# okgarces/deep-successor-features-for-transfer

Measured on AMD Instinct MI355X. Metric: env steps/sec (whole node), Reacher 8-task SF-DQN at 1/2/4/8 MI355X, higher is better.
Workload: dtype fp32; 1 GPU; reacher17-all-T8-B32 (Reacher-shape |s|=17 |a|=7 d=8, psi MLP 256x2, all heads updated per env step: main_sfdqn_torch.py path); heads_per_gpu=8, heads_total=8, global_batch=32, replay=host, parallelism=single

## Files before the change

deep-successor-features-for-transfer_amd/csrc/sfx.hip:

```cpp
#include <hip/hip_ext.h>
#include <hip/hip_runtime.h>
#include <dlfcn.h>
#include <rccl/rccl.h>

#include <cmath>
#include <cstdio>
#include <cstdlib>
#include <cstring>
#include <algorithm>
#include <atomic>
#include <chrono>
#include <deque>
#include <map>
#include <random>
#include <string>
#include <functional>
#include <tuple>
#include <utility>
#include <vector>

#include "sfx_kernels.h"
#include "sfx_gpiw.h"
#include "sfx_tsf.h"
#include "sfx_phi.h"
// ... 140 lines not shown
    const float *S = nullptr, *S1 = nullptr, *phi = nullptr, *gamma = nullptr, *s_next = nullptr;
    const int64_t* a = nullptr;
    float* losses = nullptr;
    bool pre = false;
    const float* ax = nullptr;
    int aM = 0;
    bool posted = false;
    float* q_out = nullptr;
    int64_t* task_out = nullptr;
    const unsigned long long* out_ind = nullptr;
  } pend;
  long long steps_spec = 0, steps_fallback = 0, policies_rerun = 0, rounds_total = 0;
  long long graph_captures = 0, graph_launches = 0;
  int force_rerun_from = -1;
  int spec_rounds = 2;
  bool spec_rounds_auto = true;
  int Tg = 0, off = 0;
  struct sfx_tsf_state* tsf = nullptr;
  struct sfx_phi_state* phi = nullptr;
  int comm_rank = 0, comm_world = 0;
  ncclComm_t comm = nullptr;
  bool comm_owned = false;
  ncclComm_t comm_rounds = nullptr;
  bool rounds_comm = false;
  bool comm_dead = false;
  std::string comm_err;
  long long* dstall = nullptr;
  bool comm_force = false;
  int (*host_ar)(void*, int32_t*, int) = nullptr;
  void* host_ar_ctx = nullptr;
  int32_t* host_ar_buf = nullptr;
  size_t host_ar_cap = 0;
  int *xb[2] = {nullptr, nullptr}, *xge = nullptr;
  int *tsx = nullptr, *tsz = nullptr;
  int *qh = nullptr, *qhs = nullptr;
  bool shard_qa = true;
  struct ShardPending {
    bool active = false;
    int B = 0;
    const float *S = nullptr, *S1 = nullptr, *phi = nullptr, *gamma = nullptr, *s_next = nullptr;
    const int64_t* a = nullptr;
  } spend;

  float *online = nullptr, *target = nullptr, *am = nullptr, *av = nullptr;
  float *w = nullptr, *wm = nullptr, *wv = nullptr;
  int* step = nullptr;
  int* dcancel = nullptr;
  AdamC* adamc = nullptr;
  float *act = nullptr, *dz = nullptr, *rowloss = nullptr;
  int64_t* spec_next = nullptr;
  int* skip = nullptr;
  unsigned long long* skipc = nullptr;
  bool skip_rounds = true;
  StepOut* dout = nullptr;
  HostResult* pub_res = nullptr;
  const long long* pub_dctr = nullptr;
  bool pub_folded = false;
  bool fold_publish = true;
  bool bf16 = false;
  __bf16* on16 = nullptr;
  __bf16* tg16 = nullptr;
  int dxs_max = 1, dx_ntile = 1;
  float* dxpart = nullptr;
  unsigned* dxctr = nullptr;
  StepOut* hout = nullptr;
  bool post_hout = false, hout_posted = false;
  unsigned long long* xin = nullptr;
  hipEvent_t ev_step = nullptr;
  unsigned long long gen = 0;
  int in_runner = 0;

  int slot(int head) const { return (int)((mask >> head) & 1ull); }
  unsigned long long all_bits() const { return T >= 64 ? ~0ull : ((1ull << T) - 1ull); }
  float* online_cur(int head) const { return online + ((size_t)slot(head) * T + head) * P; }
  float* am_cur(int head) const { return am + ((size_t)slot(head) * T + head) * P; }
  float* av_cur(int head) const { return av + ((size_t)slot(head) * T + head) * P; }
  float* target_of(int head) const { return target + (size_t)head * P; }
  __bf16* on16_cur(int head) const { return on16 + ((size_t)slot(head) * T + head) * P; }
  __bf16* tg16_of(int head) const { return tg16 + (size_t)head * P; }
};

namespace {

inline void touch(sfx_handle* h) {
  if (!h->in_runner) ++h->gen;
}

void clear_graphs(sfx_handle* h) {
  for (auto& kv : h->graphs) (void)hipGraphExecDestroy(kv.second);
  h->graphs.clear();
  h->graph_posts.clear();
}

enum { K_FWD = 0, K_TDG = 1, K_BWD = 2, K_GPI = 3, K_LMS = 4, K_VER = 5, K_TSF = 6, K_NKIND = 7 };

hipEvent_t prof_event(sfx_handle* h) {
  if (!h->prof_pool.empty()) {
    hipEvent_t e = h->prof_pool.back();
    h->prof_pool.pop_back();
    return e;
  }
  hipEvent_t e = nullptr;
  (void)hipEventCreate(&e);
  return e;
}

// ... 342 lines not shown
  A.tdg_next = td.next;
  A.tdg_xmax = td.xmax;
  A.tdg_poloff = td.poloff;
  A.flag = td.flag;
  A.flag_value = h->T;
  A.dz_scale = td.dz_scale;
  if (armed && fuse) {
    A.tdg_prev = td.prev;
    A.skip = h->skip;
    A.skipc = h->skipc;
    A.skip_v0 = ex.skip_fwd ? 1 : 0;
  }
  if (armed) {
    A.skip = h->skip;
    A.skip_v0 = ex.skip_fwd ? 1 : 0;
  }
  if (ex.skip_armed) *ex.skip_armed = armed;
  const int tail_at = fuse ? 1 : 0;
  const bool need_tail = losses || r || !fuse;
  const double tdg_bytes = 4.0 * nhead * M * ((td.use_gpi ? h->T : 1) * h->O + 2.0 * h->O + 2.0 * h->d + 4);
  A.M = M;
  A.head0 = head0;
  A.mask = h->mask;
  A.hp = h->hp_psi;
  A.hpw = h->hp_w;
  A.x0 = x0;
  A.phi = phi;
  A.r = r;
  A.train_w = r != nullptr;
  A.losses = losses;
  A.inc_step = ex.inc_step;
  auto dw_tiles = [&](int l) { return cdiv(h->L[l].N, 32) * cdiv(h->L[l].K, 64); };
  auto geo = [&](int l) {
    const LayerGeo& L = h->L[l];
    RoleGeo r{};
    r.N = L.N;
    r.K = L.K;
    r.wOff = L.wOff;
    r.bOff = L.bOff;
    r.actIn = L.actIn;
    r.xOff = l == 0 ? -1 : h->actOff[l - 1];
    r.dzOff = h->actOff[l];
    r.dzIn = l == 0 ? 0 : h->actOff[l - 1];
    return r;
  };
  auto dx_bytes = [&](int l) {
    const LayerGeo& L = h->L[l];
    return 4.0 * ((double)L.N * L.K + (double)M * L.N + 2.0 * M * L.K);
  };
  auto dw_bytes = [&](int l) {
    const LayerGeo& L = h->L[l];
    return 24.0 * ((double)L.N * L.K + L.N) + 4.0 * ((double)M * L.N + (double)M * L.K);
  };
  for (int l = h->NL - 1; l >= 1; --l) {
    const int li = h->NL - 1 - l;
    A.tdg = fuse && li == 0 ? 1 : 0;
    A.xi_src = A.tdg ? td.xi_src : nullptr;
    A.xi_dst = A.tdg ? td.xi_dst : nullptr;
    A.xi_copy = td.xi_copy;
    A.xi_n = td.xi_n;
    const double by = nhead * (dx_bytes(l) + (l + 1 <= h->NL - 1 ? dw_bytes(l + 1) : 0.0)) + (A.tdg ? tdg_bytes : 0.0);
    A.ra = geo(l);
    A.na = cdiv(M, 32) * cdiv(h->L[l].K, 16);
    A.dxs = 1;
    if (!A.tdg && h->dxpart && h->L[l].N > DX_SPLIT_N && M <= 32 * cdiv(h->Mmax, 32) &&
        nhead <= h->T) {
      A.dxs = cdiv(h->L[l].N, DX_SPLIT_N);
      A.dxpart = h->dxpart;
      A.dxctr = h->dxctr;
      A.na *= A.dxs;
    }
    if (l + 1 <= h->NL - 1) {
      A.rb = geo(l + 1);
      A.nb = dw_tiles(l + 1);
    } else {
      A.nb = 0;
    }
    A.nc = 0;
    A.tail = li == tail_at && need_tail ? 1 : 0;
    const int ntile = A.tdg ? A.na : A.na + A.nb + A.nc + A.tail;
    const dim3 grid = A.xcd ? dim3(8 * cdiv(nhead, 8) * ntile) : dim3(ntile, nhead);
    if (A.tdg && tdg_variant(h) == 1)
      launch(h, K_BWD, by, k_bwd_tdg<2, 8>, grid, dim3(256), h->G, A);
    else if (A.tdg)
      launch(h, K_BWD, by, k_bwd_tdg<4, 4>, grid, dim3(256), h->G, A);
    else if (!(ex.ride && nhead == 1 && !A.xcd && ex.ride(li, tail_at, A, ntile, by)))
      launch(h, K_BWD, by, h->bf16 ? k_bwd<true> : k_bwd<false>, grid, dim3(256), h->G, A);
  }
  A.na = 0;
  A.dxs = 1;
  A.tdg = 0;
  A.xi_dst = nullptr;
  A.xi_src = nullptr;
  A.rb = geo(1);
  A.nb = dw_tiles(1);
  A.rc = geo(0);
  A.nc = dw_tiles(0);
  A.tail = h->NL - 1 == tail_at && need_tail ? 1 : 0;
  A.fuse_v0 = ex.fuse_v0 ? 1 : 0;
  A.vM = M + (ex.v_xn ? 1 : 0);
  A.vOff = h->actOff[0];
  A.vRole = ex.vRole;
  A.act0 = h->L[0].actOut;
  A.v_x = ex.v_x;
  A.v_xn = ex.v_xn;
  A.ax = ex.fuse_v0 ? ex.ax : nullptr;
  A.aM = ex.fuse_v0 && ex.ax ? ex.aM : 0;
  A.a_noskip = ex.a_noskip;
  const int ntile = A.nb + A.nc + A.tail;
  if (!(ex.ride && nhead == 1 && !A.xcd && ex.ride(h->NL - 1, tail_at, A, ntile, nhead * (dw_bytes(1) + dw_bytes(0)))))
    launch(h, K_BWD, nhead * (dw_bytes(1) + dw_bytes(0)), h->bf16 ? k_bwd<true> : k_bwd<false>,
           A.xcd ? dim3(8 * cdiv(nhead, 8) * ntile) : dim3(ntile, nhead), dim3(256), h->G, A);
  LAUNCHCHK();
  return SFX_OK;
}

GpiArgs gpi_args(int role, int rowoff, int row0, const float* w, float* psi, float* q, int64_t* task, int64_t* next,
                 int64_t* sel, int select_task, int use_gpi, int M) {
  GpiArgs A{};
  A.M = M;
  A.role = role;
  A.row0 = row0;
  A.rowoff = rowoff;
  A.select_task = select_task;
  A.use_gpi = use_gpi;
  A.w = w;
  A.psi_out = psi;
  A.q_out = q;
  A.task_out = task;
  A.next_out = next;
  A.sel_out = sel;
  return A;
}

int run_gpi(sfx_handle* h, const GpiArgs& A) {
  launch(h, K_GPI, 4.0 * A.M * ((double)h->T * h->O * (A.psi_out ? 2 : 1) + h->d + (A.q_out ? h->T * h->A : 0)),
         k_gpi, dim3(A.M), dim3(256), h->G, A);
  LAUNCHCHK();
  return SFX_OK;
}

int run_ver(sfx_handle* h, int M, int npol, bool sel, int post, const GpiArgs& g, const int64_t* spec,
            bool post_host = false) {
  VerArgs V{};
  V.M = M;
  V.post = post;
  V.npol = npol;
  V.sel = sel ? 1 : 0;
  V.spec_stride = MMAX;
  V.spec_next = spec;
  V.flag = &h->dout->flag;
  V.g = g;
  const int TA = h->T * h->A;
  V.rows = TA >= 256 ? 1 : (256 / TA < M ? 256 / TA : M);
  const bool wide = wide_gpi(h) && npol > 1;
  const dim3 grid = wide ? dim3(M, cdiv(npol, WPC) + 1) : dim3(npol + 1, cdiv(M, V.rows));
  if (sel && h->pub_res && h->fold_publish) {
    V.pub = h->pub_res;
    V.pub_dctr = h->pub_dctr;
    V.done = &h->dout->done;
    V.nblocks = (int)(grid.x * grid.y);
    h->pub_folded = true;
  } else if (post_host) {
    V.h_sel = h->hout->sel;
// ... 483 lines not shown
  unsigned n = 0;
  if (hipDeviceSynchronize() != hipSuccess) return -1;
  if (hipMemcpyFromSymbol(&n, HIP_SYMBOL(sfx::g_probe_n), sizeof(n)) != hipSuccess) return -1;
  if (n > sfx::PROBE_N) n = sfx::PROBE_N;
  if ((int)n > max_recs) n = (unsigned)max_recs;
  if (n && hipMemcpyFromSymbol(out_host, HIP_SYMBOL(sfx::g_probe), n * sizeof(sfx::ProbeRec)) != hipSuccess) return -1;
  const unsigned z = 0;
  if (hipMemcpyToSymbol(HIP_SYMBOL(sfx::g_probe_n), &z, sizeof(z)) != hipSuccess) return -1;
  return (int)n;
}
#endif

int sfx_create(sfx_t* out, int T, int n_s, int H, int n_hidden, const int* acts, int A, int d, int max_batch,
               int device, void* stream) {
  if (!out) SFX_FAIL(SFX_E_ARG, "out is null");
  *out = nullptr;
  if (T < 1 || T > 64 || n_s < 1 || H < 1 || n_hidden < 0 || n_hidden + 2 > NLMAX || A < 1 || d < 1 ||
      max_batch < 1)
    SFX_FAIL(SFX_E_ARG, "bad geometry (1 <= T <= 64 heads per handle)");
  if (d > DMAX || max_batch + 1 > MMAX || (long)T * A > QMAX || (long)A * d > OMAX)
    SFX_FAIL(SFX_E_ARG, "geometry exceeds kernel limits (d<=256, batch<1024, T*A<=8192, A*d<=4096)");
  for (int i = 0; i < n_hidden; ++i)
    if (!acts || acts[i] < ACT_NONE || acts[i] > ACT_TANH) SFX_FAIL(SFX_E_ARG, "bad activation code");
  HIPCHK(hipSetDevice(device));
  sfx_handle* h = new sfx_handle();
  h->T = T;
  h->n_s = n_s;
  h->H = H;
  h->nh = n_hidden;
  h->A = A;
  h->d = d;
  h->O = A * d;
  h->NL = n_hidden + 2;
  h->Mmax = max_batch;
  h->device = device;
  h->stream = (hipStream_t)stream;
  h->dpad = align4(d);
  const char* eg = std::getenv("SFX_GRAPHS");
  h->use_graphs = !(eg && eg[0] == '0');
  const char* efp = std::getenv("SFX_FOLD_PUBLISH");
  h->fold_publish = !(efp && efp[0] == '0');
  {
    int dev = 0, ncu = 0;
    if (hipGetDevice(&dev) == hipSuccess &&
        hipDeviceGetAttribute(&ncu, hipDeviceAttributeMultiprocessorCount, dev) == hipSuccess && ncu > 0)
      h->ncu = ncu;
  }
  const char* etp = std::getenv("SFX_FWD_TPW");
  h->fwd_tpw = etp && etp[0] == '1' ? 1 : FWD_TPW;
  const char* eqa = std::getenv("SFX_SHARD_QA");
  h->shard_qa = !(eqa && eqa[0] == '0');
  const char* esk = std::getenv("SFX_SKIP");
  h->skip_rounds = !(esk && esk[0] == '0');
  int off = 0, ptorch = 0;
  for (int l = 0; l < h->NL; ++l) {
    LayerGeo Lr{};
    if (l == 0) {
      Lr.N = H; Lr.K = n_s; Lr.actOut = ACT_NONE;
    } else if (l == h->NL - 1) {
      Lr.N = h->O; Lr.K = H; Lr.actOut = ACT_NONE;
    } else {
      Lr.N = H; Lr.K = H; Lr.actOut = acts[l - 1];
    }
    Lr.actIn = l > 0 ? h->L[l - 1].actOut : ACT_NONE;
    Lr.wOff = align8(off);
    off = Lr.wOff + Lr.N * Lr.K;
    Lr.bOff = align4(off);
    off = Lr.bOff + Lr.N;
    ptorch += Lr.N * Lr.K + Lr.N;
    h->L.push_back(Lr);
  }
  h->P = (off + 63) & ~63;
  h->Ptorch = ptorch;
  int aoff = 0;
  for (int l = 0; l < h->NL; ++l) {
    h->actOff.push_back(aoff);
    aoff += align4((max_batch + 1) * h->L[l].N);
  }
  h->actSize = (aoff + 63) & ~63;
  h->Tg = T;
  h->spec_rounds = auto_spec_rounds(T);
  h->since_target.assign(T, 0);
  h->host_step.assign(T, 0);

  const size_t headBytes = sizeof(float) * (size_t)T * h->P;
  const size_t wBytes = sizeof(float) * (size_t)T * h->dpad;
  int rc = SFX_OK;
  auto alloc = [&](void** p, size_t bytes) {
    if (rc != SFX_OK) return;
    if (hipMalloc(p, bytes) != hipSuccess || hipMemset(*p, 0, bytes) != hipSuccess) {
      g_err = "hipMalloc failed";
      rc = SFX_E_HIP;
    }
  };
  alloc((void**)&h->online, 2 * headBytes);
  alloc((void**)&h->target, headBytes);
  alloc((void**)&h->am, 2 * headBytes);
  alloc((void**)&h->av, 2 * headBytes);
  alloc((void**)&h->w, wBytes);
  alloc((void**)&h->wm, wBytes);
  alloc((void**)&h->wv, wBytes);
  alloc((void**)&h->step, sizeof(int) * T);
  alloc((void**)&h->dcancel, 64);
  alloc((void**)&h->adamc, sizeof(AdamC) * T);
  {
    int nmax = 0, kmax = 0;
// ... 655 lines not shown
```

deep-successor-features-for-transfer_amd/csrc/sfx_kernels.h:

```cpp
#pragma once
#include <hip/hip_runtime.h>
#include <stdint.h>

#include <type_traits>

namespace sfx {

typedef float floatx4 __attribute__((ext_vector_type(4)));

constexpr int NLMAX = 8;
constexpr int MT = 32;
constexpr int QMAX = 8192;
constexpr int OMAX = 4096;
constexpr int DMAX = 256;
constexpr int MMAX = 1024;
constexpr int KFUSE = 64;
constexpr int GEMV_N = 512;
constexpr int GEMV_M = 4;
constexpr int DX_SPLIT_N = 256;
constexpr int VFUSE = 4096;
constexpr int TQF = 4096;

enum { ACT_NONE = 0, ACT_RELU = 1, ACT_TANH = 2 };
enum { R_S = 0, R_S1T = 1, R_S1 = 2, R_G = 3, R_A = 4, R_V = 5, R_V2 = 6, R_NS = 7, R_NS1T = 8, R_NS1 = 9, NROLE = 10 };
// ... 957 lines not shown
  float* grow = G.dzp(pol, NLm) + (size_t)b * O;
  const float* crow = G.actp(R_S, pol, NLm) + (size_t)b * O;
  const int an = s_next;
  for (int o = tid; o < O; o += 256) {
    float gv = 0.f;
    if (aok && o >= ab * d && o < ab * d + d) {
      const int k = o - ab * d;
      const float tg = __fadd_rn(A.phi[(size_t)b * d + k], __fmul_rn(gam, s_t[an * d + k]));
      gv = td_grad(G.huber, norm, __fsub_rn(crow[o], tg));
    }
    grow[o] = gv;
  }
  float dsq = 0.f;
  if (tid < d && aok) {
    const float diff = __fsub_rn(cval, __fadd_rn(phik, __fmul_rn(gam, s_t[an * d + tid])));
    dsq = td_loss(G.huber, diff);
    if (!__builtin_isfinite(diff) && G.nonfin) atomicOr(G.nonfin, 1);
  }
  if (tid < d) s_sq[tid] = dsq;
  __syncthreads();
  if (tid == 0) {
    float s = 0.f;
    for (int k = 0; k < d; ++k) s = __fadd_rn(s, s_sq[k]);
    SFX_CHK(pol >= 0 && pol < G.T && b < MMAX, pol, b, 0);
    G.rowloss[(long long)pol * MMAX + b] = s;
  }
  PROBE_REC(17, pt0);
}

struct RoleGeo {
  int N, K, wOff, bOff, actIn;
  int xOff;
  int dzOff;
  int dzIn;
};

struct BwdArgs {
  int M, na, nb, nc, tail, head0, train_w, inc_step;
  int xcd, nhead;
  int step_in_tail;
  int tdg, tdg_use_gpi, tdg_guess, tdg_next_stride, flag_value, pad2_;
  const int64_t* tdg_a;
  const float* tdg_gamma;
  int64_t* tdg_next;
  const int* tdg_xmax;
  int tdg_poloff, pad3_;
  int* flag;
  int fuse_v0, vM, vOff, act0;
  int vRole, dxs;
  unsigned long long mask;
  float* dxpart;
  unsigned* dxctr;
  RoleGeo ra, rb, rc;
  AdamHP hp, hpw;
  const float* x0;
  const float* phi;
  const float* r;
  float* losses;
  const float* v_x;
  const float* v_xn;
  const float* ax;
  int aM, a_noskip;
  const int* xi_src;
  int* xi_dst;
  int xi_copy, xi_n;
  const int64_t* tdg_prev;
  int* skip;
  unsigned long long* skipc;
  int skip_v0, pad4_;
  const float* dz_scale;
};

__device__ __forceinline__ const float* layer_input(const Geo& G, const BwdArgs& A, int head, int xOff) {
  return xOff < 0 ? A.x0 : G.actp(R_S, head, xOff);
}

constexpr int TDG_ROWS_O = 128;
struct TdgSmem {
  float w[32], gam[32], ph[32 * 16];
  int a[32], n[32];
  float q[2048], m[32 * 128];
  float tt[32 * TDG_ROWS_O], tc[32 * TDG_ROWS_O];
  float dz[32 * TDG_ROWS_O];
};

template <int VMAX, int U, bool C>
__device__ int tdg_rows(const Geo& G, const BwdArgs& A, int pol, int m0, bool pub, TdgSmem& sm) {
  const int tid = threadIdx.x, T = G.T, Aa = G.A, d = G.d, O = G.O, NLm = G.lastOff, M = A.M;
  const int nb = M - m0 < 32 ? M - m0 : 32;
  const bool xm = A.tdg_xmax != nullptr;
  const int t0 = A.tdg_use_gpi ? 0 : pol, nt = A.tdg_use_gpi ? T : 1, TA = nt * Aa, n = xm ? 0 : nb * TA, V = d >> 2;
  const int guess = A.tdg_guess;
  const FDiv fTA = fdiv(TA), fA = fdiv(Aa);
  float4 v[U][VMAX];
#pragma unroll
  for (int u = 0; u < U; ++u) {
    const int idx = tid + u * 256;
    const bool ok = idx < n;
    const int bl = idx / fTA, rem = idx - bl * TA, tq = rem / fA, t = t0 + tq, a = rem - tq * Aa;
    const float4* p = reinterpret_cast<const float4*>(G.actp(t < pol ? guess : R_S1, ok ? t : 0, NLm) +
                                                      (ok ? (size_t)(m0 + bl) * O + a * d : 0));
#pragma unroll
    for (int j = 0; j < VMAX; ++j) v[u][j] = (ok && j < V) ? p[j] : make_float4(0.f, 0.f, 0.f, 0.f);
  }
  const int n4 = (nb * O) >> 2;
  const float4* tg4 = reinterpret_cast<const float4*>(G.actp(R_S1T, pol, NLm) + (size_t)m0 * O);
  const float4* cu4 = reinterpret_cast<const float4*>(G.actp(R_S, pol, NLm) + (size_t)m0 * O);
  float4 tt[4], tc[4];
#pragma unroll
  for (int u = 0; u < 4; ++u) {
    const int i = tid + u * 256;
    tt[u] = i < n4 ? tg4[i] : make_float4(0.f, 0.f, 0.f, 0.f);
    tc[u] = i < n4 ? cu4[i] : make_float4(0.f, 0.f, 0.f, 0.f);
  }
  const int np4 = (nb * d) >> 2;
  const float4 ph = tid < np4 ? reinterpret_cast<const float4*>(A.phi + (size_t)m0 * d)[tid] : make_float4(0.f, 0.f, 0.f, 0.f);
  const float wk = tid < d ? G.w[(long long)pol * G.dpad + tid] : 0.f;
  const int ab_l = tid < nb ? (int)A.tdg_a[m0 + tid] : 0;
  const float gam_l = tid < nb ? A.tdg_gamma[m0 + tid] : 0.f;
  int xv[4];
  if (xm) {
    const int* xr = A.tdg_xmax + ((size_t)(A.tdg_poloff + pol) * M + m0) * Aa;
// ... 67 lines not shown
    if (pub && A.tdg_next) A.tdg_next[(size_t)(pol - A.head0) * A.tdg_next_stride + m0 + bl] = am;
  }
  const int same = !__syncthreads_or(differs);
  if (pub && A.skip && tid == 0) {
    A.skip[pol] = same;
    if (A.skipc && prev) {
      atomicAdd(A.skipc, 1ull);
      if (same) atomicAdd(A.skipc + 1, 1ull);
    }
  }
  if (same) return 1;
  PROBE_AT(4);
  const float norm = td_norm(G, M, O, A.dz_scale);
  const FDiv fd = fdiv(d);
  float* sq = sm.q;
  int nf = 0;
  for (int i = tid; i < nb * d; i += 256) {
    const int bl = i / fd, k = i - bl * d, ab = sm.a[bl];
    float e2 = 0.f;
    if (ab >= 0 && ab < Aa) {
      const float tg = __fadd_rn(sm.ph[bl * d + k], __fmul_rn(sm.gam[bl], sm.tt[bl * O + sm.n[bl] * d + k]));
      const float diff = __fsub_rn(sm.tc[bl * O + ab * d + k], tg);
      sm.dz[bl * O + ab * d + k] = td_grad(G.huber, norm, diff);
      e2 = td_loss(G.huber, diff);
      nf |= !__builtin_isfinite(diff);
    }
    sq[i] = e2;
  }
  if (__syncthreads_or(nf) && tid == 0 && G.nonfin) atomicOr(G.nonfin, 1);
  PROBE_AT(7);
  if (pub) {
    float4* gout4 = reinterpret_cast<float4*>(G.dzp(pol, NLm) + (size_t)m0 * O);
    for (int i = tid; i < n4; i += 256) {
      const float4 v = reinterpret_cast<const float4*>(sm.dz)[i];
      if constexpr (C) {
        float* o = reinterpret_cast<float*>(gout4 + i);
        stc<true>(o, v.x);
        stc<true>(o + 1, v.y);
        stc<true>(o + 2, v.z);
        stc<true>(o + 3, v.w);
      } else {
        gout4[i] = v;
      }
    }
    for (int bl = tid; bl < nb; bl += 256) {
      float sacc = 0.f;
      for (int k = 0; k < d; ++k) sacc = __fadd_rn(sacc, sq[bl * d + k]);
      SFX_CHK(pol >= 0 && pol < G.T && m0 + bl < MMAX, pol, m0 + bl, 0);
      G.rowloss[(long long)pol * MMAX + m0 + bl] = sacc;
    }
  }
  PROBE_AT(8);
  return 0;
}

template <bool TDG, int VMAX = 2, int U = 8, bool C = false, bool BF = false>
__device__ __forceinline__ void role_dx(const Geo& G, const BwdArgs& A, int head, int tile, floatx4 (*red)[2][64]) {
  static_assert(!(BF && (TDG || C)), "bf16 dX: the plain dX tiles only (the fused TD launch stays fp32)");
  const RoleGeo L = A.ra;
  const int N = L.N, K = L.K, M = A.M;
  const int ntk = (K + 15) >> 4;
  const int split = TDG ? 0 : tile % A.dxs;
  tile = TDG ? tile : tile / A.dxs;
  const int nchunk = ((N + A.dxs - 1) / A.dxs + 63) & ~63;
  const int nbeg = split * nchunk, nend = min(N, nbeg + nchunk);
  const int k0 = (tile % ntk) * 16, m0 = (tile / ntk) * 32;
  const int wave = threadIdx.x >> 6, lane = threadIdx.x & 63, r = lane & 15, g = lane >> 4;
  const float* W = G.online + G.slot_off(rslot(A.mask, head), head) + L.wOff;
  const float* Xin = layer_input(G, A, head, L.xOff);
  float* out = G.dzp(head, L.dzIn);
  const int ma = m0 + r, mb = m0 + 16 + r, kk = k0 + r;
  const bool oka = ma < M, okb = mb < M, okk = kk < K;
  const int s = (threadIdx.x >> 6) & 1, Lx = threadIdx.x & 63, col = k0 + (Lx & 15);
  float xin[4] = {0.f, 0.f, 0.f, 0.f};
  if (threadIdx.x < 128 && col < K) {
#pragma unroll
    for (int i = 0; i < 4; ++i) {
      const int row = m0 + 16 * s + (Lx >> 4) * 4 + i;
      if (row < M) xin[i] = Xin[(size_t)row * K + col];
    }
  }
  floatx4 acc0 = {0.f, 0.f, 0.f, 0.f}, acc1 = {0.f, 0.f, 0.f, 0.f};
  if constexpr (TDG) {
    __shared__ TdgSmem sm;
    if (tile == 0 && A.inc_step && threadIdx.x == 0 && !step_cancelled(G.cancel)) {
      const int st = G.step[head] + 1;
      const AdamC ac = adam_consts(A.hp, st);
      if constexpr (C) {
        __hip_atomic_store(G.step + head, st, __ATOMIC_RELAXED, __HIP_MEMORY_SCOPE_AGENT);
        float* f = reinterpret_cast<float*>(G.adamc + head);
        stc<true>(f, ac.omb1);
        stc<true>(f + 1, ac.b2);
        stc<true>(f + 2, ac.omb2);
        stc<true>(f + 3, ac.eps);
        stc<true>(f + 4, ac.wd);
        stc<true>(f + 5, ac.bc2s);
        stc<true>(f + 6, ac.nss);
      } else {
        G.step[head] = st;
        G.adamc[head] = ac;
      }
    }
    if (A.flag && tile == 0 && head == A.head0 && threadIdx.x == 0) *A.flag = A.flag_value;
    const int wpc = N > 64 ? 2 : 4, jw = 16 / wpc, j0 = (wave % wpc) * jw;
    const int nb = (wave / wpc) * 64 + g * 16;
    float bw[16];
#pragma unroll
    for (int j = 0; j < 16; ++j)
      bw[j] = (j >= j0 && j < j0 + jw && okk && nb + j < N) ? W[(size_t)(nb + j) * K + kk] : 0.f;
    if (tdg_rows<VMAX, U, C>(G, A, head, m0, tile % ntk == 0, sm)) return;
    const float* da = sm.dz + (size_t)r * N + nb;
    const float* db = sm.dz + (size_t)(16 + r) * N + nb;
#pragma unroll
    for (int j = 0; j < 16; ++j) {
      if (j >= j0 && j < j0 + jw) {
        const bool okj = nb + j < N;
        acc0 = mfma4(oka && okj ? da[j] : 0.f, bw[j], acc0);
        acc1 = mfma4(okb && okj ? db[j] : 0.f, bw[j], acc1);
      }
    }
  } else {
    const float* dZ = G.dzp(head, L.dzOff);
    const bool vec = (N & 63) == 0;
    for (int nc = nbeg + wave * 64; nc < nend; nc += 256) {
      const int nb = nc + g * 16;
      float a0[16], a1[16], bw[16];
      load16u<C>(a0, dZ + (size_t)ma * N, nb, nend, oka, vec);
      load16u<C>(a1, dZ + (size_t)mb * N, nb, nend, okb, vec);
      if constexpr (BF) {
        const __bf16* W16 = G.on16 + G.slot_off(rslot(A.mask, head), head) + L.wOff;
        bf16x8 w16[2];
#pragma unroll
        for (int j = 0; j < 16; ++j)
          w16[j >> 3][j & 7] = (okk && nb + j < nend) ? W16[(size_t)(nb + j) * K + kk] : (__bf16)0.f;
#pragma unroll
        for (int s2 = 0; s2 < 2; ++s2) {
          acc0 = mfma_bf16(to_bf16x8(a0 + 8 * s2), w16[s2], acc0);
          acc1 = mfma_bf16(to_bf16x8(a1 + 8 * s2), w16[s2], acc1);
        }
        continue;
      }
#pragma unroll
      for (int j = 0; j < 16; ++j) bw[j] = (okk && nb + j < nend) ? W[(size_t)(nb + j) * K + kk] : 0.f;
#pragma unroll
      for (int j = 0; j < 16; ++j) {
        acc0 = mfma4(a0[j], bw[j], acc0);
        acc1 = mfma4(a1[j], bw[j], acc1);
      }
    }
  }
  PROBE_MARK();
  red[wave][0][lane] = acc0;
  red[wave][1][lane] = acc1;
  __syncthreads();
  if (!TDG && A.dxs > 1) {
    const int ntile = ((M + 31) >> 5) * ntk;
    const size_t pt = ((size_t)(head - A.head0) * ntile + tile) * A.dxs;
    __shared__ int s_last;
    if (threadIdx.x < 128) {
      floatx4 v = red[0][s][Lx];
      v += red[1][s][Lx];
      v += red[2][s][Lx];
      v += red[3][s][Lx];
      float* o = A.dxpart + ((pt + split) * 128 + threadIdx.x) * 4;
#ifdef SFX_CHECK
      SFX_CHK((long long)((pt + split) * 128 + threadIdx.x) * 4 + 3 < G.ext_dxpart, pt, split, G.ext_dxpart);
#endif
#pragma unroll
      for (int i = 0; i < 4; ++i) stc<true>(o + i, v[i]);
      asm volatile("s_waitcnt vmcnt(0)" ::: "memory");
    }
    __syncthreads();
    if (threadIdx.x == 0) {
      unsigned* ctr = A.dxctr + (size_t)(head - A.head0) * ntile + tile;
      const unsigned prev = __hip_atomic_fetch_add(ctr, 1u, __ATOMIC_RELAXED, __HIP_MEMORY_SCOPE_AGENT);
      s_last = prev == (unsigned)A.dxs - 1;
      if (s_last) __hip_atomic_store(ctr, 0u, __ATOMIC_RELAXED, __HIP_MEMORY_SCOPE_AGENT);
    }
    __syncthreads();
    if (!s_last || threadIdx.x >= 128) return;
    floatx4 v = {0.f, 0.f, 0.f, 0.f};
    for (int q = 0; q < A.dxs; ++q) {
      const float* o = A.dxpart + ((pt + q) * 128 + threadIdx.x) * 4;
#pragma unroll
      for (int i = 0; i < 4; ++i) v[i] = __fadd_rn(v[i], ldc<true>(o + i));
    }
    if (col < K) {
#pragma unroll
      for (int i = 0; i < 4; ++i) {
        const int row = m0 + 16 * s + (Lx >> 4) * 4 + i;
        if (row < M) {
          G.chk_act(L.dzIn, (long long)row * K + col);
          stc<C>(out + (size_t)row * K + col, act_bwd(v[i], xin[i], L.actIn));
        }
      }
    }
    return;
  }
  if (threadIdx.x < 128) {
    floatx4 v = red[0][s][Lx];
    v += red[1][s][Lx];
    v += red[2][s][Lx];
    v += red[3][s][Lx];
    if (col < K) {
#pragma unroll
      for (int i = 0; i < 4; ++i) {
        const int row = m0 + 16 * s + (Lx >> 4) * 4 + i;
        if (row < M) {
          G.chk_act(L.dzIn, (long long)row * K + col);
          stc<C>(out + (size_t)row * K + col, act_bwd(v[i], xin[i], L.actIn));
        }
      }
    }
  }
}

__device__ __forceinline__ int v0_aoff(const BwdArgs& A, int K) { return (A.vM * K + 3) & ~3; }
constexpr int V0S = KFUSE + 4;

template <bool C>
__device__ __forceinline__ void v0_tile(const float* x, int K, int m0, int rows, const float* w, float bb, int act,
                                        float* Y, int N, int n, long long lim) {
  constexpr int KS = 8;
  const int lane = threadIdx.x & 63, r = lane & 15, g = lane >> 4, ma = m0 + r;
  floatx4 c = {0.f, 0.f, 0.f, 0.f};
  for (int k0 = 0; k0 < K; k0 += 4 * KS) {
    float a[KS], b[KS];
#pragma unroll
    for (int q = 0; q < KS; ++q) {
      const int k = k0 + 4 * q + g;
      a[q] = (k < K && ma < rows) ? x[ma * K + k] : 0.f;
      b[q] = k < K ? w[k] : 0.f;
    }
#pragma unroll
    for (int q = 0; q < KS; ++q)
      if (k0 + 4 * q < K) c = mfma4(a[q], b[q], c);
  }
  if (n < N) {
#pragma unroll
    for (int i = 0; i < 4; ++i) {
      const int m = m0 + g * 4 + i;
      if (m < rows) {
        SFX_CHK((long long)m * N + n < lim, m, n, lim);
        stc<C>(Y + (size_t)m * N + n, act_fwd(__fadd_rn(c[i], bb), act));
      }
    }
  }
}

template <bool C>
__device__ __forceinline__ void fused_v0(const Geo& G, const BwdArgs& A, const RoleGeo& L, int head, int nbase, const float* sW,
                         const float* sB, const float* sX, const float* sWt = nullptr, const float* sBt = nullptr,
                         bool vrows = true, bool landed = false) {
  if (A.aM > 0 && !landed) asm volatile("s_waitcnt vmcnt(0)" ::: "memory");
  __syncthreads();
  PROBE_AT(3);
// ... 32 lines not shown
    const float* p = j < n ? src(j) : nullptr;
    if (p)
      __builtin_amdgcn_global_load_lds((const void*)p, (tsf_lds_t)(dst + c * 64), 4, 0, 0);
    else if (j < n)
      dst[j] = 0.f;
  }
}

struct V0Smem {
  float sW[32 * V0S];
  float sB[32];
  float sWt[32 * KFUSE];
  float sBt[32];
  __align__(16) float sX[VFUSE];
};
__device__ __forceinline__ V0Smem& v0_smem() {
  __shared__ V0Smem sm;
  return sm;
}

__device__ __forceinline__ void v0_stage_ahead(const Geo& G, const BwdArgs& A, const RoleGeo& L, int head, int nbase,
                                               V0Smem& sm) {
  const int K = L.K, ncol = L.N - nbase < 32 ? L.N - nbase : 32;
  const float* ax = A.ax;
  glds(sm.sX + v0_aoff(A, K), 2 * A.aM * K, [&](int j) -> const float* { return ax + j; });
  const float* Pt = G.target + (long long)head * G.P;
  const float* tw = Pt + L.wOff + (size_t)nbase * K;
  glds(sm.sWt, 32 * K, [&](int j) -> const float* { return j < ncol * K ? tw + j : nullptr; });
  const float* tb = Pt + L.bOff + nbase;
  glds(sm.sBt, 32, [&](int j) -> const float* { return j < ncol ? tb + j : nullptr; }, 0, 1);
}

__device__ __forceinline__ void role_v0_only(const Geo& G, const BwdArgs& A, int head, const RoleGeo& L, int tile, bool vrows) {
  const int N = L.N, K = L.K, M = A.M, tid = threadIdx.x, nbase = tile * 32;
  const float* Pw = G.online + G.slot_off(rslot(A.mask, head) ^ 1, head);
  V0Smem& sm = v0_smem();
  float* sW = sm.sW;
  float* sB = sm.sB;
  float* sX = sm.sX;
  if (A.aM > 0) v0_stage_ahead(G, A, L, head, nbase, sm);
  const FDiv fK = fdiv(K);
  for (int j = tid; j < 32 * K; j += 256) {
    const int nl = j / fK, k = j - nl * K;
    sW[nl * V0S + k] = nbase + nl < N ? Pw[L.wOff + (size_t)(nbase + nl) * K + k] : 0.f;
  }
  if (tid < 32) sB[tid] = nbase + tid < N ? Pw[L.bOff + nbase + tid] : 0.f;
  if (vrows) {
    const int nxs = A.vM * K;
    for (int j = tid; j < nxs; j += 256) sX[j] = j < M * K ? A.v_x[j] : A.v_xn[j - M * K];
  }
  fused_v0<false>(G, A, L, head, nbase, sW, sB, sX, sm.sWt, sm.sBt, vrows);
}

template <bool C = false, bool BF = false>
__device__ __forceinline__ void role_dw(const Geo& G, const BwdArgs& A, int head, const RoleGeo& L, int tile, bool fuse) {
  const int N = L.N, K = L.K, M = A.M;
  const int ntk = (K + 63) >> 6;
  const int kt = tile % ntk, nt = tile / ntk;
  const int wave = threadIdx.x >> 6, lane = threadIdx.x & 63, r = lane & 15, g = lane >> 4;
  const int nbase = nt * 32, n0 = nbase + (wave & 1) * 16, k0 = kt * 64 + (wave >> 1) * 32;
  const float* dZ = G.dzp(head, L.dzOff);
  const float* X = layer_input(G, A, head, L.xOff);
  const int rs = rslot(A.mask, head);
  const long long ro = G.slot_off(rs, head), wo = G.slot_off(rs ^ 1, head);
  const float* Pr = G.online + ro;
  const float* Mr = G.am + ro;
  const float* Vr = G.av + ro;
  float* Pw = G.online + wo;
  float* Mw = G.am + wo;
  float* Vw = G.av + wo;
  const AdamC c = load_adamc<C>(G.adamc + head);
  const int cx = step_cancelled(G.cancel);
  const int nn = n0 + r, kb0 = k0 + r, kb1 = k0 + 16 + r;
  float pp[8], pm[8], pv[8];
  bool ok[8];
#pragma unroll
  for (int i = 0; i < 4; ++i) {
    const int n = n0 + g * 4 + i;
#pragma unroll
    for (int h = 0; h < 2; ++h) {
      const int k = h ? kb1 : kb0;
      const int e = i * 2 + h;
      ok[e] = n < N && k < K;
      const size_t off = (size_t)L.wOff + (size_t)n * K + k;
      pp[e] = ok[e] ? Pr[off] : 0.f;
      pm[e] = ok[e] ? Mr[off] : 0.f;
      pv[e] = ok[e] ? Vr[off] : 0.f;
    }
  }
  const bool dob = kt == 0 && wave < 2 && g == 0 && nn < N;
  const int nbias = nn;
  float bp = 0.f, bm = 0.f, bv = 0.f;
  if (dob) {
    bp = Pr[L.bOff + nbias];
    bm = Mr[L.bOff + nbias];
    bv = Vr[L.bOff + nbias];
  }
  constexpr int XQ = VFUSE / 1024;
  float4 xs[XQ];
  float xn = 0.f;
  const int nx = fuse ? M * K : 0;
  const int nxn = fuse && A.v_xn ? K : 0;
  if (fuse && A.aM > 0) v0_stage_ahead(G, A, L, head, nbase, v0_smem());
  if (fuse) {
    if ((nx & 3) == 0 && (reinterpret_cast<uintptr_t>(A.v_x) & 15) == 0) {
#pragma unroll
      for (int q = 0; q < XQ; ++q) {
        const int j = threadIdx.x + 256 * q;
        xs[q] = 4 * j < nx ? reinterpret_cast<const float4*>(A.v_x)[j] : make_float4(0.f, 0.f, 0.f, 0.f);
      }
    } else {
#pragma unroll
      for (int q = 0; q < XQ; ++q) {
        const int j = 4 * (threadIdx.x + 256 * q);
        xs[q].x = j < nx ? A.v_x[j] : 0.f;
        xs[q].y = j + 1 < nx ? A.v_x[j + 1] : 0.f;
        xs[q].z = j + 2 < nx ? A.v_x[j + 2] : 0.f;
        xs[q].w = j + 3 < nx ? A.v_x[j + 3] : 0.f;
      }
    }
    if ((int)threadIdx.x < nxn) xn = A.v_xn[threadIdx.x];
  }
  __builtin_amdgcn_sched_barrier(0);
  floatx4 acc0 = {0.f, 0.f, 0.f, 0.f}, acc1 = {0.f, 0.f, 0.f, 0.f};
  float bsum = 0.f;
  for (int mc = 0; mc < M; mc += MT) {
    float av[MT / 4], bv0[MT / 4], bv1[MT / 4];
#pragma unroll
    for (int j = 0; j < MT / 4; ++j) {
      const int m = mc + 4 * j + g;
      const bool okm = m < M;
      av[j] = (okm && nn < N) ? ldc<C>(dZ + (size_t)m * N + nn) : 0.f;
      bv0[j] = (okm && kb0 < K) ? X[(size_t)m * K + kb0] : 0.f;
      bv1[j] = (okm && kb1 < K) ? X[(size_t)m * K + kb1] : 0.f;
    }
#pragma unroll
    for (int j = 0; j < MT / 4; ++j) {
      acc0 = mfma4(av[j], bv0[j], acc0);
      acc1 = mfma4(av[j], bv1[j], acc1);
    }
#pragma unroll
    for (int j = 0; j < MT / 4; ++j) bsum = __fadd_rn(bsum, av[j]);
  }
  bsum = __fadd_rn(bsum, __shfl_xor(bsum, 16));
  bsum = __fadd_rn(bsum, __shfl_xor(bsum, 32));
  if (fuse && A.aM > 0) asm volatile("s_waitcnt vmcnt(0)" ::: "memory");
  PROBE_MARK();
  V0Smem& sm = v0_smem();
  float* sW = sm.sW;
  float* sB = sm.sB;
  float* sX = sm.sX;
  if (fuse) {
#pragma unroll
    for (int q = 0; q < XQ; ++q) {
      const int j = threadIdx.x + 256 * q;
      if (4 * j + 3 < nx) {
        reinterpret_cast<float4*>(sX)[j] = xs[q];
      } else if (4 * j < nx) {
        sX[4 * j] = xs[q].x;
        if (4 * j + 1 < nx) sX[4 * j + 1] = xs[q].y;
        if (4 * j + 2 < nx) sX[4 * j + 2] = xs[q].z;
      }
    }
    if ((int)threadIdx.x < nxn) sX[nx + threadIdx.x] = xn;
  }
#pragma unroll
  for (int i = 0; i < 4; ++i) {
    const int n = n0 + g * 4 + i;
#pragma unroll
    for (int h = 0; h < 2; ++h) {
      const int e = i * 2 + h;
      if (ok[e]) {
        const int k = h ? kb1 : kb0;
        const size_t off = (size_t)L.wOff + (size_t)n * K + k;
        SFX_CHK((long long)off < G.P, L.wOff, n, k);
        adam_apply(pp[e], pm[e], pv[e], h ? acc1[i] : acc0[i], c);
        if (!cx) {
          st_param<C>(Pw + off, pp[e]);
          st_moment(Mw + off, pm[e]);
          st_moment(Vw + off, pv[e]);
          if constexpr (BF) G.on16[wo + off] = (__bf16)pp[e];
        }
        if (fuse) sW[(n - nbase) * V0S + k] = pp[e];
      }
// ... 27 lines not shown

__device__ __forceinline__ void role_tail(const Geo& G, const BwdArgs& A, int head) {
  const int M = A.M, d = G.d, tid = threadIdx.x;
  __shared__ float s_e[MMAX];
  __shared__ float s_red[256];
  __shared__ float s_phi[2048];
  const int step = A.step_in_tail && A.inc_step ? G.step[head] + 1 : G.step[head];
  const int cx = step_cancelled(G.cancel);
  const float* rl = G.rowloss + (long long)head * MMAX;
  float* w = G.w + (long long)head * G.dpad;
  float part = 0.f;
  for (int b = tid; b < M; b += 256) part = __fadd_rn(part, rl[b]);
  float l2 = 0.f;
  if (A.train_w) {
    const bool lds_phi = M * d <= 2048;
    if (lds_phi)
      for (int j = tid; j < M * d; j += 256) s_phi[j] = A.phi[j];
    __syncthreads();
    const float* ph = lds_phi ? s_phi : A.phi;
    float se = 0.f;
    for (int b = tid; b < M; b += 256) {
      float rf = 0.f;
      for (int k = 0; k < d; ++k) rf = __builtin_fmaf(w[k], ph[(size_t)b * d + k], rf);
      s_e[b] = __fsub_rn(rf, A.r[b]);
      se = __builtin_fmaf(s_e[b], s_e[b], se);
    }
    se = block_sum(se, s_red);
    const AdamC c = adam_consts(A.hpw, step);
    const float nrm = (float)(2.0 / (double)M);
    float gw = 0.f;
    if (tid < d) {
      for (int b = 0; b < M; ++b) gw = __builtin_fmaf(__fmul_rn(nrm, s_e[b]), ph[(size_t)b * d + tid], gw);
    }
    __syncthreads();
    if (tid < d && !cx) adam_el(w + tid, G.wm + (long long)head * G.dpad + tid, G.wv + (long long)head * G.dpad + tid, gw, c);
    l2 = (float)((double)se / (double)M);
  }
  const float s = A.losses ? block_sum(part, s_red) : 0.f;
  if (tid == 0) {
    const float l1 = (float)((double)s / ((double)M * (double)G.O));
    if (A.losses) {
      float* lo = A.losses + 3 * (head - A.head0);
      lo[0] = __fadd_rn(l1, l2);
      lo[1] = l1;
      lo[2] = l2;
    }
    if (A.step_in_tail && !cx) {
      G.step[head] = step;
      G.adamc[head] = adam_consts(A.hp, step);
    }
  }
}

template <bool BF>
__device__ __forceinline__ void bwd_body(const Geo& G, const BwdArgs& A, int head, int bx, floatx4 (*red)[2][64]) {
  PROBE_T(pt0);
  PROBE_MARKA();
  const bool skip = A.skip && __builtin_nontemporal_load(A.skip + head) != 0;
  if (bx < A.nc) {
    if (skip) {
      if (A.fuse_v0 && (!A.skip_v0 || (A.aM > 0 && A.a_noskip))) role_v0_only(G, A, head, A.rc, bx, !A.skip_v0);
      return;
    }
    role_dw<false, BF>(G, A, head, A.rc, bx, A.fuse_v0 != 0);
    PROBE_REC(6, pt0);
    return;
  }
  bx -= A.nc;
  if (bx < A.nb) {
    if (skip) return;
    role_dw<false, BF>(G, A, head, A.rb, bx, false);
    PROBE_REC(5, pt0);
    return;
  }
  bx -= A.nb;
  if (bx < A.na) {
    if (skip) return;
    role_dx<false, 2, 8, false, BF>(G, A, head, bx, red);
    PROBE_REC(4, pt0);
    return;
  }
  role_tail(G, A, head);
}

template <bool BF = false>
__global__ __launch_bounds__(256) void k_bwd(Geo G, BwdArgs A) {
  __shared__ floatx4 red[4][2][64];
  int head = A.head0 + blockIdx.y, bx = blockIdx.x;
  if (A.xcd) {
    if (!xcd_decode(blockIdx.x, A.nhead, A.na + A.nb + A.nc + A.tail, head, bx)) return;
    head += A.head0;
  }
  bwd_body<BF>(G, A, head, bx, red);
}

template <int VMAX, int U>
__global__ __launch_bounds__(256) void k_bwd_tdg(Geo G, BwdArgs A) {
  __shared__ floatx4 red[4][2][64];
  PROBE_T(pt0);
  if (A.xi_dst)
    fill_sortable(A.xi_dst, A.xi_src, A.xi_copy, A.xi_n, (blockIdx.y * gridDim.x + blockIdx.x) * 256 + threadIdx.x,
                  gridDim.x * gridDim.y * 256);
  int head = A.head0 + blockIdx.y, bx = blockIdx.x;
  if (A.xcd) {
    if (!xcd_decode(blockIdx.x, A.nhead, A.na, head, bx)) return;
    head += A.head0;
  }
  PROBE_MARKA();
  role_dx<true, VMAX, U>(G, A, head, bx, red);
  PROBE_REC(3, pt0);
}

struct GpiArgs {
  int M, role, row0, select_task, use_gpi, rowoff;
  int w_stride, sel_stride;
  const float* w;
  float* psi_out;
  float* q_out;
  int64_t* task_out;
  int64_t* next_out;
  int64_t* sel_out;
  const unsigned long long* out_ind;
};

__device__ __forceinline__ unsigned long long argmax_key(float v, int idx) {
  const unsigned int u = __float_as_uint(__fadd_rn(v, 0.f));
  const unsigned int o = (u & 0x80000000u) ? ~u : (u | 0x80000000u);
  return ((unsigned long long)o << 32) | (unsigned long long)(0xFFFFFFFFu - (unsigned)idx);
}
__device__ __forceinline__ int argmax_idx(unsigned long long key) { return (int)(0xFFFFFFFFu - (unsigned)(key & 0xFFFFFFFFull)); }
__device__ __forceinline__ unsigned long long wave_max(unsigned long long k) {
#pragma unroll
  for (int m = 32; m >= 1; m >>= 1) {
    const unsigned long long o = __shfl_xor(k, m, 64);
    k = o > k ? o : k;
  }
  return k;
}

__device__ __forceinline__ int gpi_pick(const GpiArgs& A, const float* s_q, float* s_mt, float* s_ma, int T, int Aa,
                                        long long ob, int64_t* so, int nthr) {
  const int tid = threadIdx.x;
  for (int t = tid; t < T; t += nthr) {
    float mx = s_q[t * Aa];
    for (int a = 1; a < Aa; ++a) mx = fmaxf(mx, s_q[t * Aa + a]);
    s_mt[t] = mx;
// ... 847 lines not shown
```

Baseline: 8140 env steps/s.

## Merge layer-1 dX into the final backward launch via per-tile recompute

Result: faster. 8305 env steps/s (median of 6 runs) (+2.0%).

```diff
diff --git a/deep-successor-features-for-transfer_amd/csrc/sfx.hip b/deep-successor-features-for-transfer_amd/csrc/sfx.hip
--- a/deep-successor-features-for-transfer_amd/csrc/sfx.hip
+++ b/deep-successor-features-for-transfer_amd/csrc/sfx.hip
@@ -216,6 +216,7 @@
   int* skip = nullptr;
   unsigned long long* skipc = nullptr;
   bool skip_rounds = true;
+  bool bwd_merge = true;
   StepOut* dout = nullptr;
   HostResult* pub_res = nullptr;
   const long long* pub_dctr = nullptr;
@@ -664,7 +665,9 @@
     const LayerGeo& L = h->L[l];
     return 24.0 * ((double)L.N * L.K + L.N) + 4.0 * ((double)M * L.N + (double)M * L.K);
   };
-  for (int l = h->NL - 1; l >= 1; --l) {
+  const bool merge = h->bwd_merge && nhead > 1 && !ex.ride && h->NL >= 3 && M <= 32 && ex.fuse_v0 &&
+                     can_fuse_v0(h, M + (ex.v_xn ? 1 : 0)) && h->L[1].N <= DX_SPLIT_N;
+  for (int l = h->NL - 1; l >= (merge ? 2 : 1); --l) {
     const int li = h->NL - 1 - l;
     A.tdg = fuse && li == 0 ? 1 : 0;
     A.xi_src = A.tdg ? td.xi_src : nullptr;
@@ -708,7 +711,16 @@
   A.nb = dw_tiles(1);
   A.rc = geo(0);
   A.nc = dw_tiles(0);
-  A.tail = h->NL - 1 == tail_at && need_tail ? 1 : 0;
+  const int last = merge ? h->NL - 2 : h->NL - 1;
+  A.tail = last == tail_at && need_tail ? 1 : 0;
+  double by_last = nhead * (dw_bytes(1) + dw_bytes(0));
+  if (merge) {
+    A.merge = 1;
+    A.ra = geo(1);
+    A.rd = geo(2);
+    A.nd = dw_tiles(2);
+    by_last += nhead * (dw_bytes(2) + dx_bytes(1) - 4.0 * M * h->L[1].K - 4.0 * M * h->L[0].N);
+  }
   A.fuse_v0 = ex.fuse_v0 ? 1 : 0;
   A.vM = M + (ex.v_xn ? 1 : 0);
   A.vOff = h->actOff[0];
@@ -719,9 +731,12 @@
   A.ax = ex.fuse_v0 ? ex.ax : nullptr;
   A.aM = ex.fuse_v0 && ex.ax ? ex.aM : 0;
   A.a_noskip = ex.a_noskip;
-  const int ntile = A.nb + A.nc + A.tail;
-  if (!(ex.ride && nhead == 1 && !A.xcd && ex.ride(h->NL - 1, tail_at, A, ntile, nhead * (dw_bytes(1) + dw_bytes(0)))))
-    launch(h, K_BWD, nhead * (dw_bytes(1) + dw_bytes(0)), h->bf16 ? k_bwd<true> : k_bwd<false>,
+  const int ntile = A.nb + A.nc + A.nd + A.tail;
+  if (merge)
+    launch(h, K_BWD, by_last, h->bf16 ? k_bwd_mg<true> : k_bwd_mg<false>, dim3(8 * cdiv(nhead, 8) * ntile), dim3(256),
+           h->G, A);
+  else if (!(ex.ride && nhead == 1 && !A.xcd && ex.ride(h->NL - 1, tail_at, A, ntile, by_last)))
+    launch(h, K_BWD, by_last, h->bf16 ? k_bwd<true> : k_bwd<false>,
            A.xcd ? dim3(8 * cdiv(nhead, 8) * ntile) : dim3(ntile, nhead), dim3(256), h->G, A);
   LAUNCHCHK();
   return SFX_OK;
@@ -1311,6 +1326,8 @@
   h->shard_qa = !(eqa && eqa[0] == '0');
   const char* esk = std::getenv("SFX_SKIP");
   h->skip_rounds = !(esk && esk[0] == '0');
+  const char* ebm = std::getenv("SFX_BWD_MERGE");
+  h->bwd_merge = !(ebm && ebm[0] == '0');
   int off = 0, ptorch = 0;
   for (int l = 0; l < h->NL; ++l) {
     LayerGeo Lr{};
diff --git a/deep-successor-features-for-transfer_amd/csrc/sfx_kernels.h b/deep-successor-features-for-transfer_amd/csrc/sfx_kernels.h
--- a/deep-successor-features-for-transfer_amd/csrc/sfx_kernels.h
+++ b/deep-successor-features-for-transfer_amd/csrc/sfx_kernels.h
@@ -1033,6 +1033,8 @@
   float* dxpart;
   unsigned* dxctr;
   RoleGeo ra, rb, rc;
+  RoleGeo rd;
+  int nd, pad5_;
   AdamHP hp, hpw;
   const float* x0;
   const float* phi;
@@ -1048,7 +1050,8 @@
   const int64_t* tdg_prev;
   int* skip;
   unsigned long long* skipc;
-  int skip_v0, pad4_;
+  int skip_v0;
+  int merge;
   const float* dz_scale;
 };
 
@@ -1222,6 +1225,74 @@
   }
   PROBE_AT(8);
   return 0;
+}
+
+template <bool BF, int NS>
+struct DxOps {
+  float a0[16], a1[16];
+  float bw[BF ? 1 : NS][16];
+  bf16x8 w16[BF ? NS : 1][2];
+};
+
+template <bool C, bool BF, int NS>
+__device__ __forceinline__ void dx_load(DxOps<BF, NS>& o, const float* dZ, const float* W, const __bf16* W16, int N, int K,
+                                        int nc, int nend, int ma, int mb, bool oka, bool okb, const int (&kk)[NS]) {
+  const int nb = nc + ((threadIdx.x & 63) >> 4) * 16;
+  const bool vec = (N & 63) == 0, in = nc < nend;
+  load16u<C>(o.a0, dZ + (size_t)ma * N, nb, nend, oka && in, vec);
+  load16u<C>(o.a1, dZ + (size_t)mb * N, nb, nend, okb && in, vec);
+#pragma unroll
+  for (int s = 0; s < NS; ++s) {
+#pragma unroll
+    for (int j = 0; j < 16; ++j) {
+      const bool ok = kk[s] < K && nb + j < nend;
+      if constexpr (BF) o.w16[s][j >> 3][j & 7] = ok ? W16[(size_t)(nb + j) * K + kk[s]] : (__bf16)0.f;
+      else o.bw[s][j] = ok ? W[(size_t)(nb + j) * K + kk[s]] : 0.f;
+    }
+  }
+}
+
+template <bool BF, int NS>
+__device__ __forceinline__ void dx_mma(const DxOps<BF, NS>& o, floatx4 (&acc)[NS][2]) {
+  if constexpr (BF) {
+#pragma unroll
+    for (int s2 = 0; s2 < 2; ++s2) {
+      const bf16x8 x0 = to_bf16x8(o.a0 + 8 * s2), x1 = to_bf16x8(o.a1 + 8 * s2);
+#pragma unroll
+      for (int s = 0; s < NS; ++s) {
+        acc[s][0] = mfma_bf16(x0, o.w16[s][s2], acc[s][0]);
+        acc[s][1] = mfma_bf16(x1, o.w16[s][s2], acc[s][1]);
+      }
+    }
+  } else {
+#pragma unroll
+    for (int j = 0; j < 16; ++j) {
+#pragma unroll
+      for (int s = 0; s < NS; ++s) {
+        acc[s][0] = mfma4(o.a0[j], o.bw[s][j], acc[s][0]);
+        acc[s][1] = mfma4(o.a1[j], o.bw[s][j], acc[s][1]);
+      }
+    }
+  }
+}
+
+template <bool C, bool BF, int NS>
+__device__ __forceinline__ void dx_accum(const float* dZ, const float* W, const __bf16* W16, int N, int K, int nbeg,
+                                         int nend, int ma, int mb, bool oka, bool okb, const int (&kk)[NS],
+                                         floatx4 (&acc)[NS][2]) {
+  for (int nc = nbeg + (threadIdx.x >> 6) * 64; nc < nend; nc += 256) {
+    DxOps<BF, NS> o;
+    dx_load<C, BF, NS>(o, dZ, W, W16, N, K, nc, nend, ma, mb, oka, okb, kk);
+    dx_mma<BF, NS>(o, acc);
+  }
+}
+
+__device__ __forceinline__ floatx4 dx_red_sum(const floatx4 (*red)[2][64], int s, int Lx) {
+  floatx4 v = red[0][s][Lx];
+  v += red[1][s][Lx];
+  v += red[2][s][Lx];
+  v += red[3][s][Lx];
+  return v;
 }
 
 template <bool TDG, int VMAX = 2, int U = 8, bool C = false, bool BF = false>
@@ -1290,34 +1361,12 @@
       }
     }
   } else {
-    const float* dZ = G.dzp(head, L.dzOff);
-    const bool vec = (N & 63) == 0;
-    for (int nc = nbeg + wave * 64; nc < nend; nc += 256) {
-      const int nb = nc + g * 16;
-      float a0[16], a1[16], bw[16];
-      load16u<C>(a0, dZ + (size_t)ma * N, nb, nend, oka, vec);
-      load16u<C>(a1, dZ + (size_t)mb * N, nb, nend, okb, vec);
-      if constexpr (BF) {
-        const __bf16* W16 = G.on16 + G.slot_off(rslot(A.mask, head), head) + L.wOff;
-        bf16x8 w16[2];
-#pragma unroll
-        for (int j = 0; j < 16; ++j)
-          w16[j >> 3][j & 7] = (okk && nb + j < nend) ? W16[(size_t)(nb + j) * K + kk] : (__bf16)0.f;
-#pragma unroll
-        for (int s2 = 0; s2 < 2; ++s2) {
-          acc0 = mfma_bf16(to_bf16x8(a0 + 8 * s2), w16[s2], acc0);
-          acc1 = mfma_bf16(to_bf16x8(a1 + 8 * s2), w16[s2], acc1);
-        }
-        continue;
-      }
-#pragma unroll
-      for (int j = 0; j < 16; ++j) bw[j] = (okk && nb + j < nend) ? W[(size_t)(nb + j) * K + kk] : 0.f;
-#pragma unroll
-      for (int j = 0; j < 16; ++j) {
-        acc0 = mfma4(a0[j], bw[j], acc0);
-        acc1 = mfma4(a1[j], bw[j], acc1);
-      }
-    }
+    const int kks[1] = {kk};
+    floatx4 acc[1][2] = {{acc0, acc1}};
+    dx_accum<C, BF, 1>(G.dzp(head, L.dzOff), W, BF ? G.on16 + G.slot_off(rslot(A.mask, head), head) + L.wOff : nullptr, N, K,
+                       nbeg, nend, ma, mb, oka, okb, kks, acc);
+    acc0 = acc[0][0];
+    acc1 = acc[0][1];
   }
   PROBE_MARK();
   red[wave][0][lane] = acc0;
@@ -1328,10 +1377,7 @@
     const size_t pt = ((size_t)(head - A.head0) * ntile + tile) * A.dxs;
     __shared__ int s_last;
     if (threadIdx.x < 128) {
-      floatx4 v = red[0][s][Lx];
-      v += red[1][s][Lx];
-      v += red[2][s][Lx];
-      v += red[3][s][Lx];
+      const floatx4 v = dx_red_sum(red, s, Lx);
       float* o = A.dxpart + ((pt + split) * 128 + threadIdx.x) * 4;
 #ifdef SFX_CHECK
       SFX_CHK((long long)((pt + split) * 128 + threadIdx.x) * 4 + 3 < G.ext_dxpart, pt, split, G.ext_dxpart);
@@ -1368,10 +1414,7 @@
     return;
   }
   if (threadIdx.x < 128) {
-    floatx4 v = red[0][s][Lx];
-    v += red[1][s][Lx];
-    v += red[2][s][Lx];
-    v += red[3][s][Lx];
+    const floatx4 v = dx_red_sum(red, s, Lx);
     if (col < K) {
 #pragma unroll
       for (int i = 0; i < 4; ++i) {
@@ -1510,8 +1553,9 @@
   fused_v0<false>(G, A, L, head, nbase, sW, sB, sX, sm.sWt, sm.sBt, vrows);
 }
 
-template <bool C = false, bool BF = false>
-__device__ __forceinline__ void role_dw(const Geo& G, const BwdArgs& A, int head, const RoleGeo& L, int tile, bool fuse) {
+template <bool C = false, bool BF = false, bool MG = false>
+__device__ __forceinline__ void role_dw(const Geo& G, const BwdArgs& A, int head, const RoleGeo& L, int tile, bool fuse,
+                                        floatx4 (*red)[2][64] = nullptr) {
   const int N = L.N, K = L.K, M = A.M;
   const int ntk = (K + 63) >> 6;
   const int kt = tile % ntk, nt = tile / ntk;
@@ -1582,12 +1626,54 @@
   __builtin_amdgcn_sched_barrier(0);
   floatx4 acc0 = {0.f, 0.f, 0.f, 0.f}, acc1 = {0.f, 0.f, 0.f, 0.f};
   float bsum = 0.f;
+  float dz0[MT / 4], xb0[MT / 4], xb1[MT / 4];
+  if constexpr (MG) {
+    static_assert(MT == 32, "merged tile: the 32 rows of one dX tile are the one row chunk of dW");
+    __shared__ floatx4 red2[4][2][64];
+    const RoleGeo& L1 = A.ra;
+    const float* Y0 = layer_input(G, A, head, L1.xOff);
+    float y0[MT / 4];
+#pragma unroll
+    for (int j = 0; j < MT / 4; ++j) {
+      const int m = 4 * j + g;
+      y0[j] = (m < M && nn < N) ? Y0[(size_t)m * N + nn] : 0.f;
+      xb0[j] = (m < M && kb0 < K) ? X[(size_t)m * K + kb0] : 0.f;
+      xb1[j] = (m < M && kb1 < K) ? X[(size_t)m * K + kb1] : 0.f;
+    }
+    const int kks[2] = {nbase + r, nbase + 16 + r};
+    floatx4 dacc[2][2] = {};
+    dx_accum<false, BF, 2>(G.dzp(head, L1.dzOff), Pr + L1.wOff, BF ? G.on16 + ro + L1.wOff : nullptr, L1.N, L1.K, 0, L1.N, r,
+                           16 + r, r < M, 16 + r < M, kks, dacc);
+    red[wave][0][lane] = dacc[0][0];
+    red[wave][1][lane] = dacc[0][1];
+    red2[wave][0][lane] = dacc[1][0];
+    red2[wave][1][lane] = dacc[1][1];
+    PROBE_AT(6);
+    __syncthreads();
+    const floatx4 (*rd)[2][64] = (wave & 1) ? red2 : red;
+#pragma unroll
+    for (int j = 0; j < MT / 4; ++j) {
+      const int s = j >> 2, Lx = (j & 3) * 16 + r;
+      float v = rd[0][s][Lx][g];
+      v = __fadd_rn(v, rd[1][s][Lx][g]);
+      v = __fadd_rn(v, rd[2][s][Lx][g]);
+      v = __fadd_rn(v, rd[3][s][Lx][g]);
+      dz0[j] = (4 * j + g < M && nn < N) ? act_bwd(v, y0[j], L1.actIn) : 0.f;
+    }
+    PROBE_AT(7);
+  }
   for (int mc = 0; mc < M; mc += MT) {
     float av[MT / 4], bv0[MT / 4], bv1[MT / 4];
 #pragma unroll
     for (int j = 0; j < MT / 4; ++j) {
       const int m = mc + 4 * j + g;
       const bool okm = m < M;
+      if constexpr (MG) {
+        av[j] = dz0[j];
+        bv0[j] = xb0[j];
+        bv1[j] = xb1[j];
+        continue;
+      }
       av[j] = (okm && nn < N) ? ldc<C>(dZ + (size_t)m * N + nn) : 0.f;
       bv0[j] = (okm && kb0 < K) ? X[(size_t)m * K + kb0] : 0.f;
       bv1[j] = (okm && kb1 < K) ? X[(size_t)m * K + kb1] : 0.f;
@@ -1721,7 +1807,7 @@
   }
 }
 
-template <bool BF>
+template <bool BF, bool MG = false>
 __device__ __forceinline__ void bwd_body(const Geo& G, const BwdArgs& A, int head, int bx, floatx4 (*red)[2][64]) {
   PROBE_T(pt0);
   PROBE_MARKA();
@@ -1731,11 +1817,18 @@
       if (A.fuse_v0 && (!A.skip_v0 || (A.aM > 0 && A.a_noskip))) role_v0_only(G, A, head, A.rc, bx, !A.skip_v0);
       return;
     }
-    role_dw<false, BF>(G, A, head, A.rc, bx, A.fuse_v0 != 0);
+    role_dw<false, BF, MG>(G, A, head, A.rc, bx, A.fuse_v0 != 0, red);
     PROBE_REC(6, pt0);
     return;
   }
   bx -= A.nc;
+  if (bx < A.nd) {
+    if (skip) return;
+    role_dw<false, BF>(G, A, head, A.rd, bx, false);
+    PROBE_REC(5, pt0);
+    return;
+  }
+  bx -= A.nd;
   if (bx < A.nb) {
     if (skip) return;
     role_dw<false, BF>(G, A, head, A.rb, bx, false);
@@ -1757,10 +1850,18 @@
   __shared__ floatx4 red[4][2][64];
   int head = A.head0 + blockIdx.y, bx = blockIdx.x;
   if (A.xcd) {
-    if (!xcd_decode(blockIdx.x, A.nhead, A.na + A.nb + A.nc + A.tail, head, bx)) return;
+    if (!xcd_decode(blockIdx.x, A.nhead, A.na + A.nb + A.nc + A.nd + A.tail, head, bx)) return;
     head += A.head0;
   }
   bwd_body<BF>(G, A, head, bx, red);
+}
+
+template <bool BF = false>
+__global__ __launch_bounds__(256) void k_bwd_mg(Geo G, BwdArgs A) {
+  __shared__ floatx4 red[4][2][64];
+  int head, bx;
+  if (!xcd_decode(blockIdx.x, A.nhead, A.na + A.nb + A.nc + A.nd + A.tail, head, bx)) return;
+  bwd_body<BF, true>(G, A, head + A.head0, bx, red);
 }
 
 template <int VMAX, int U>
```
